# apple/ml-neuman

Measured on AMD Instinct MI355X. Metric: rays_per_sec (800x800 frame, 128 samples/ray coarse + 128 importance, NeuMan background NeRF), higher is better.
Workload: dtype coarse (sampling) pass: split-fp16 hi+lo MFMA x3, f32 accumulate; fine (shading) pass: per-row-scaled int16 as two int8 limbs on the i8 MFMA x3, exact int32 accumulate, encodings on split bf16

## Files before the change

ml-neuman_amd/csrc/mlp_host.hip:

```cpp
#include <stdarg.h>
#include <stdio.h>
#include <stdlib.h>
#include <string.h>

#include <vector>

#include "common.h"
#include "mlp_layout.h"
#include "mlp_launch.h"

namespace nm {

static thread_local char g_err[512] = "";

void set_error(const char* fmt, ...) {
    va_list ap;
    va_start(ap, fmt);
    vsnprintf(g_err, sizeof(g_err), fmt, ap);
    va_end(ap);
}
int check_hip(hipError_t e, const char* what) {
    if (e == hipSuccess) return NM_OK;
    set_error("%s: %s", what, hipGetErrorString(e));
    return NM_ERR_HIP;
// ... 278 lines not shown
                const float* row = hidden_row(d, P, st, n, &col0);
                float mx = 0.f;
                if (row) for (int f = 0; f < nh; ++f) mx = fmaxf(mx, fabsf(row[col0 + f] * uin[f]));
                q[n] = mx / (float)kFixedMax;
                kap = fmaxf(kap, q[n]);
            }
            if (!(kap > 0.f)) kap = 1.f;
            kappa[st] = kap;
            for (int n = 0; n < nrows; ++n) {
                if (!(q[n] > 0.f)) q[n] = kap;
                u[n] = q[n] / kap;
            }
            for (int nb = 0; nb < sh.nblk; ++nb)
                for (int r = 0; r < 32; ++r) {
                    const int n = 32 * nb + r;
                    int col0 = 0;
                    const float* row = hidden_row(d, P, st, n, &col0);
                    for (int t = 0; t < sh.i8steps; ++t) {
                        int8_t* hi = reinterpret_cast<int8_t*>(img + frag_off8(st, nb, t));
                        int8_t* lo = hi + 1024;
                        for (int g = 0; g < 2; ++g)
                            for (int e = 0; e < 16; ++e) {
                                const int f = slot_feature8(2 * t + g, e);
                                const float w = row ? row[col0 + f] * uin[f] : 0.f;
                                int v = (int)lrintf(w / q[n]);
                                if (v > kFixedMax) v = kFixedMax;
                                if (v < -kFixedMax) v = -kFixedMax;
                                const int l = ((v + 128) & 255) - 128;
                                const int h = (v - l) >> 8;
                                hi[(g * 32 + r) * 16 + e] = (int8_t)h;
                                lo[(g * 32 + r) * 16 + e] = (int8_t)l;
                            }
                    }
                }
        }
        for (int n = 0; n < nrows; ++n) b[n] /= u[n];
        for (int nb = 0; nb < sh.nblk; ++nb)
            for (int t = 0; t < sh.bfsteps; ++t) {
                uint16_t* hi = reinterpret_cast<uint16_t*>(img + frag_off8(st, nb, sh.i8steps + t));
                uint16_t* lo = hi + 64 * 8;
                const int cc0 = st == 9 ? 32 : 0;
                for (int lane = 0; lane < 64; ++lane)
                    for (int j = 0; j < 8; ++j) {
                        const int n = 32 * nb + (lane & 31);
                        const float wv = stage_weight(d, P, st, n, cc0 + 2 * t + (lane >> 5), j) / u[n];
                        const uint16_t h = f32_to_bf16(wv);
                        hi[lane * 8 + j] = h;
                        lo[lane * 8 + j] = f32_to_bf16(wv - bf16_to_f32(h));
                    }
            }
    }
}

static void pack_stream8s(const uint8_t* img8, uint8_t* out, bool plain = false) {
    memset(out, 0, (size_t)(kWeightBytes8 + kWeightPadBytes));
    uint8_t* dst = out;
    auto put = [&](int st, int nb, int t0, int n) {
        for (int t = 0; t < n; ++t, dst += kStepBytes) memcpy(dst, img8 + frag_off8(st, nb, t0 + t), (size_t)kStepBytes);
    };
    for (int nb = 0; nb < 8; ++nb) put(0, nb, 0, 4);
    for (int st = 1; st <= 7; ++st) {
        for (int nb = 0; nb < 8; ++nb) put(st, nb, 0, 8);
        if (st == 5)
            for (int nb = 0; nb < 8; ++nb) put(5, nb, 8, 4);
    }
    put(8, 8, 0, 8);
    if (plain) {
        for (int nb = 0; nb < 2; ++nb) { put(0, nb, 0, 4); dst += 4 * kStepBytes; }
        if (dst - out != kPlainStreamBytes8) abort();
        return;
    }
    for (int nb = 0; nb < 8; ++nb) put(8, nb, 0, 8);
    for (int nb = 0; nb < 4; ++nb) put(9, nb, 0, 10);
    put(10, 0, 0, 4);
    if (dst - out != kWeightBytes8) abort();
}

constexpr int kSigmaSteps = 8 * 4 + 6 * 8 * 16 + 8 * 20 + 16;
static void sigma_stream_table(std::vector<int>& tab, int ndir) {
    tab.clear();
    std::vector<int> direct;
    auto put = [&](int st, int b, int t0, int n) {
        for (int t = 0; t < n; ++t)
            for (int k = 0; k < 4; ++k) {
                const int off = (int)frag_off(st, b + (k >> 1), t0 + t) + 1024 * (k & 1);
                (k < 4 - ndir ? tab : direct).push_back(off);
            }
    };
    for (int st = 0; st <= 7; ++st) {
        const StageShape sh = stage_shape(st);
        for (int b = 0; b < 8; b += 2) {
            if (sh.pe_steps) put(st, b, 0, sh.pe_steps);
            for (int t0 = sh.pe_steps; t0 < sh.steps; t0 += 8) put(st, b, t0, 8);
        }
    }
    for (int t = 0; t < 16; ++t) { tab.push_back((int)frag_off(8, 8, t)); tab.push_back((int)frag_off(8, 8, t) + 1024); }
    tab.insert(tab.end(), direct.begin(), direct.end());
    if ((int)tab.size() != 2 * kSigmaSteps) abort();
}
__global__ void sigma_stream_kernel(const uint4* __restrict__ image, const int* __restrict__ tab, int npieces, uint4* __restrict__ out) {
    const int i = blockIdx.x * blockDim.x + threadIdx.x;
    if (i >= npieces * 64) return;
    out[i] = image[tab[i >> 6] / 16 + (i & 63)];
}

static void pack_stream8(const uint8_t* img8, uint8_t* out) {
    memset(out, 0, (size_t)kWeightBytes8w);
    for (int q = 0; q < 4; ++q) {
        uint8_t* dst = out + wstream_off(q);
        auto put = [&](int st, int nb, int t0, int n) {
            for (int t = 0; t < n; ++t, dst += kStepBytes) memcpy(dst, img8 + frag_off8(st, nb, t0 + t), (size_t)kStepBytes);
        };
        put(0, 2 * q, 0, 4); put(0, 2 * q + 1, 0, 4);
        for (int st = 1; st <= 8; ++st) {
            put(st, 2 * q, 0, 8); put(st, 2 * q + 1, 0, 8);
            if (st == 5) { put(5, 2 * q, 8, 4); put(5, 2 * q + 1, 8, 4); }
        }
        if (q < 2) put(8, 8, 0, 8);
        put(9, q, 0, 8); put(9, q, 8, 2);
        dst += 2 * kStepBytes;
        if (q < 2) put(10, 0, 0, 4);
        dst += kW8Pad * kStepBytes;
        if (dst != out + wstream_off(q) + (int64_t)wstream_steps(q) * kStepBytes) abort();
    }
}

}
// ... 41 lines not shown

int nm_mlp_pack_f16(const nm_mlp_desc* desc, const float* const* host_params, void* host_out) {
    if (int e = nm::validate_desc(desc)) return e;
    NM_REQUIRE(host_params && host_out, "nm_mlp_pack_f16: null pointer");
    for (int i = 0; i < (desc->plain_head ? 18 : 24); ++i) NM_REQUIRE(host_params[i], "nm_mlp_pack_f16: host_params[%d] is null", i);
    nm::pack_image(desc, host_params, static_cast<uint8_t*>(host_out), true);
    return NM_OK;
}

int64_t nm_mlp_pack_i8_bytes(const nm_mlp_desc* desc) {
    if (nm::validate_desc(desc) != NM_OK) return -1;
    return nm::image8_bytes();
}

int nm_mlp_pack_i8(const nm_mlp_desc* desc, const float* const* host_params, void* host_out) {
    if (int e = nm::validate_desc(desc)) return e;
    NM_REQUIRE(host_params && host_out, "nm_mlp_pack_i8: null pointer");
    for (int i = 0; i < (desc->plain_head ? 18 : 24); ++i) NM_REQUIRE(host_params[i], "nm_mlp_pack_i8: host_params[%d] is null", i);
    nm::pack_image8(desc, host_params, static_cast<uint8_t*>(host_out));
    return NM_OK;
}

int64_t nm_mlp_pack_i8s_bytes(const nm_mlp_desc* desc) {
    if (nm::validate_desc(desc) != NM_OK) return -1;
    return nm::kWeightBytes8 + nm::kWeightPadBytes;
}

int nm_mlp_pack_i8s(const nm_mlp_desc* desc, const float* const* host_params, void* host_out) {
    if (int e = nm::validate_desc(desc)) return e;
    NM_REQUIRE(host_params && host_out, "nm_mlp_pack_i8s: null pointer");
    for (int i = 0; i < (desc->plain_head ? 18 : 24); ++i) NM_REQUIRE(host_params[i], "nm_mlp_pack_i8s: host_params[%d] is null", i);
    std::vector<uint8_t> img8((size_t)nm::image8_bytes());
    nm::pack_image8(desc, host_params, img8.data());
    nm::pack_stream8s(img8.data(), static_cast<uint8_t*>(host_out), desc->plain_head != 0);
    return NM_OK;
}

int nm_mlp_create(const nm_mlp_desc* desc, const float* const* host_params, const float* host_pos_tab,
                  const float* host_dir_tab, nm_mlp_t* out) {
    if (int e = nm::validate_desc(desc)) return e;
    NM_REQUIRE(host_params && host_pos_tab && host_dir_tab && out, "nm_mlp_create: null pointer");
    const int plain = desc->plain_head;
    for (int i = 0; i < (plain ? 18 : 24); ++i) NM_REQUIRE(host_params[i], "nm_mlp_create: host_params[%d] is null", i);
    const int64_t bytes = nm_mlp_pack_bytes(desc);
    std::vector<uint8_t> img((size_t)bytes);
    nm::pack_image(desc, host_params, img.data());
    std::vector<uint8_t> img16((size_t)bytes);
    nm::pack_image(desc, host_params, img16.data(), true);
    std::vector<uint8_t> img8((size_t)nm::image8_bytes());
    std::vector<uint8_t> str8((size_t)nm::kWeightBytes8w);
    std::vector<uint8_t> str8s((size_t)(nm::kWeightBytes8 + nm::kWeightPadBytes));
    nm::pack_image8(desc, host_params, img8.data());
    nm::pack_stream8(img8.data(), str8.data());
    nm::pack_stream8s(img8.data(), str8s.data(), plain != 0);

    const int kpe = 3 + 6 * desc->pos_n_freqs, kdpe = 3 + 6 * desc->dir_n_freqs;
    const int K[12] = {kpe, 256, 256, 256, 256, kpe + 256, 256, 256, plain ? 0 : 256 + kdpe, plain ? 0 : 256, 256, plain ? 0 : 128};
    const int N[12] = {256, 256, 256, 256, 256, 256, 256, 256, plain ? 0 : 128, plain ? 0 : 256, plain ? 4 : 1, plain ? 0 : 3};
    const int src[12] = {0, 2, 4, 6, 8, 10, 12, 14, 16, 18, plain ? (int)nm::P_OUT_W : 20, 22};
    nm_mlp_s* m = new nm_mlp_s();
    m->desc = *desc;
    int woff = 0;
    for (int l = 0; l < 12; ++l) { m->ref_off[l] = woff; woff += K[l] * N[l]; }
    int boff = woff;
    for (int l = 0; l < 12; ++l) { m->ref_boff[l] = boff; boff += N[l]; }
    std::vector<float> ref((size_t)boff);
    for (int l = 0; l < 12; ++l) {
        if (!K[l]) continue;
        const float* W = host_params[src[l]];
        for (int k = 0; k < K[l]; ++k)
            for (int n = 0; n < N[l]; ++n) ref[m->ref_off[l] + (size_t)k * N[l] + n] = W[(size_t)n * K[l] + k];
        memcpy(&ref[m->ref_boff[l]], host_params[src[l] + 1], (size_t)N[l] * 4);
    }
    float tab[192];
    memset(tab, 0, sizeof(tab));
    const int npos = desc->pe_kind == NM_PE_POSENC ? desc->pos_n_freqs : 9 * desc->pos_n_freqs;
    const int ndir = desc->pe_kind == NM_PE_POSENC ? desc->dir_n_freqs : 9 * desc->dir_n_freqs;
    memcpy(tab, host_pos_tab, (size_t)npos * 4);
    memcpy(tab + 96, host_dir_tab, (size_t)ndir * 4);
    auto octaves = [&](const float* t, int nfreq) {
        const int per = desc->pe_kind == NM_PE_POSENC ? 1 : 9;
        for (int b = 0; b + 1 < nfreq; ++b)
            for (int k = 0; k < per; ++k)
                if (t[(b + 1) * per + k] != 2.f * t[b * per + k]) return 0;
        return 1;
    };
    m->pos_octaves = octaves(tab, desc->pos_n_freqs);
    m->dir_octaves = octaves(tab + 96, desc->dir_n_freqs);

    m->d_image = nullptr; m->d_image16 = nullptr; m->d_consts8 = nullptr; m->d_stream8 = nullptr; m->d_image8 = nullptr; m->d_stream16t = nullptr; m->d_sigma_tab = nullptr; m->d_bwd_image = nullptr; m->d_petab = nullptr; m->d_ref = nullptr; m->d_wscale16 = nullptr;
    int rc = nm::check_hip(hipMalloc(&m->d_image, (size_t)bytes), "nm_mlp_create: hipMalloc(image)");
    const size_t consts_off = (size_t)(nm::kWeightBytes8 + nm::kWeightPadBytes), consts_bytes = img8.size() - consts_off;
    if (!rc) rc = nm::check_hip(hipMalloc(&m->d_consts8, consts_bytes), "nm_mlp_create: hipMalloc(consts8)");
    if (!rc) rc = nm::check_hip(hipMemcpy(m->d_consts8, img8.data() + consts_off, consts_bytes, hipMemcpyHostToDevice), "nm_mlp_create: upload consts8");
    if (!rc) rc = nm::check_hip(hipMalloc(&m->d_stream8, str8.size()), "nm_mlp_create: hipMalloc(stream8)");
    if (!rc) rc = nm::check_hip(hipMemcpy(m->d_stream8, str8.data(), str8.size(), hipMemcpyHostToDevice), "nm_mlp_create: upload stream8");
    if (!rc) rc = nm::check_hip(hipMalloc(&m->d_image8, consts_off), "nm_mlp_create: hipMalloc(image8)");
    if (!rc) rc = nm::check_hip(hipMemcpy(m->d_image8, str8s.data(), consts_off, hipMemcpyHostToDevice), "nm_mlp_create: upload image8");
    if (!rc) rc = nm::check_hip(hipMalloc(&m->d_petab, sizeof(tab)), "nm_mlp_create: hipMalloc(petab)");
    if (!rc) rc = nm::check_hip(hipMalloc(&m->d_ref, ref.size() * 4), "nm_mlp_create: hipMalloc(ref)");
    if (!rc) rc = nm::check_hip(hipMemcpy(m->d_image, img.data(), (size_t)bytes, hipMemcpyHostToDevice), "nm_mlp_create: upload image");
    if (!rc) rc = nm::check_hip(hipMalloc(&m->d_image16, (size_t)bytes), "nm_mlp_create: hipMalloc(image16)");
    if (!rc) rc = nm::check_hip(hipMemcpy(m->d_image16, img16.data(), (size_t)bytes, hipMemcpyHostToDevice), "nm_mlp_create: upload image16");
    if (!rc) rc = nm::check_hip(hipMemcpy(m->d_petab, tab, sizeof(tab), hipMemcpyHostToDevice), "nm_mlp_create: upload petab");
    if (!rc) rc = nm::check_hip(hipMemcpy(m->d_ref, ref.data(), ref.size() * 4, hipMemcpyHostToDevice), "nm_mlp_create: upload ref");
    if (!rc && !plain) {
        std::vector<int> stab;
// ... 42 lines not shown
}

int nm_mlp_destroy(nm_mlp_t m) {
    if (!m) return NM_OK;
    if (m->d_image) (void)hipFree(m->d_image);
    if (m->d_image16) (void)hipFree(m->d_image16);
    if (m->d_consts8) (void)hipFree(m->d_consts8);
    if (m->d_stream8) (void)hipFree(m->d_stream8);
    if (m->d_image8) (void)hipFree(m->d_image8);
    if (m->d_stream16t) (void)hipFree(m->d_stream16t);
    if (m->d_sigma_tab) (void)hipFree(m->d_sigma_tab);
    if (m->d_bwd_image) (void)hipFree(m->d_bwd_image);
    if (m->d_petab) (void)hipFree(m->d_petab);
    if (m->d_ref) (void)hipFree(m->d_ref);
    if (m->d_wscale16) (void)hipFree(m->d_wscale16);
    delete m;
    return NM_OK;
}

static int mlp_dispatch(nm_mlp_t m, const float* pts, const float* dirs, const float* origin, const float* direction,
                        const float* z, int64_t n, int S, int in_mode, int precision, int stop_stage, float sigma_scale,
                        float* out, float* dbg, nm_stream_t stream, void* prof = nullptr, int sigma_only = 0,
                        const nm::MlpChunk* chunk = nullptr) {
    NM_REQUIRE(m, "nm_mlp_forward: null handle");
    NM_REQUIRE(n >= 0, "nm_mlp_forward: negative n");
    NM_REQUIRE(precision == NM_PREC_FP32 || precision == NM_PREC_BF16X3 || precision == NM_PREC_BF16 || precision == NM_PREC_I8X3 ||
                   precision == NM_PREC_FP16X3,
               "nm_mlp_forward: bad precision %d", precision);
    if (n == 0) return NM_OK;
    NM_REQUIRE(!(chunk && precision == NM_PREC_FP32), "nm_mlp_forward_ray_chunk: the exact-f32 validation kernel has no chunked form");
    NM_REQUIRE(!(m->desc.plain_head && precision == NM_PREC_I8X3 && (stop_stage != -2 || dbg || prof || sigma_only)),
               "nm_mlp_forward: the plain-head (use_viewdirs=False) net's i8x3 form is the whole-network launch only (no stage-by-stage / density-only form)");
    NM_REQUIRE(!(m->desc.plain_head && stop_stage > 7), "nm_mlp_forward_debug: the plain-head net has stages -1..7 only");
    if (precision == NM_PREC_FP32) {
        nm::RefLaunch L;
        L.plain_head = m->desc.plain_head;
        L.wt = m->d_ref; L.bias = m->d_ref; L.petab = m->d_petab;
        for (int i = 0; i < 12; ++i) { L.off[i] = m->ref_off[i]; L.boff[i] = m->ref_boff[i]; }
        L.pe_kind = m->desc.pe_kind; L.pos_nfreq = m->desc.pos_n_freqs; L.dir_nfreq = m->desc.dir_n_freqs;
        return nm::launch_mlp_ref(L, pts, dirs, origin, direction, z, n, S, in_mode, stop_stage, sigma_scale, out, dbg,
                                  nm::as_stream(stream));
    }
    nm::MlpLaunch L;
    L.wpack = m->d_image;
    L.bias = reinterpret_cast<const float*>(m->d_image + nm::kWeightBytes + nm::kWeightPadBytes);
    L.wpack16 = m->d_image16;
    L.bias16 = reinterpret_cast<const float*>(m->d_image16 + nm::kWeightBytes + nm::kWeightPadBytes);
    L.petab = m->d_petab;
    L.pe_kind = m->desc.pe_kind; L.pos_nfreq = m->desc.pos_n_freqs; L.dir_nfreq = m->desc.dir_n_freqs;
    L.pos_octaves = m->pos_octaves; L.dir_octaves = m->dir_octaves;
    L.plain_head = m->desc.plain_head;
    L.wstream8 = m->d_stream8;
    L.consts8 = m->d_consts8;
    static const bool i8_as = [] { const char* e = getenv("NEUMAN_I8_KERNEL"); return !e || !strcmp(e, "as"); }();
    const char* sk = getenv("NEUMAN_SIGMA_KERNEL");
    const bool sigma_t = !(sk && !strcmp(sk, "w")) && m->d_stream16t;
    if (sigma_t && precision == NM_PREC_FP16X3 && sigma_only == 1 && stop_stage == -2 && !dbg && !prof && !m->desc.plain_head)
        return nm::launch_sigma_f16t(L, m->d_stream16t, m->sigma_ndir, pts, dirs, origin, direction, z, n, S, in_mode, sigma_scale, out, nm::as_stream(stream), chunk, nullptr, -1);
    if ((i8_as || m->desc.plain_head) && precision == NM_PREC_I8X3 && stop_stage == -2 && !dbg && !prof && !sigma_only)
        return nm::launch_mlp_i8s(L, m->d_image8, pts, dirs, origin, direction, z, n, S, in_mode, sigma_scale, out, nm::as_stream(stream), chunk);
    return nm::launch_mlp_mfma(L, pts, dirs, origin, direction, z, n, S, in_mode, precision, stop_stage, sigma_scale, out, dbg,
                               prof, nm::as_stream(stream), sigma_only, chunk);
}

int nm_mlp_forward(nm_mlp_t mlp, const float* pts, const float* dirs, int64_t n, int precision, float sigma_scale,
                   float* out, nm_stream_t stream) {
    NM_REQUIRE(n == 0 || (pts && dirs && out), "nm_mlp_forward: null pointer");
    NM_REQUIRE((reinterpret_cast<uintptr_t>(out) & 15) == 0, "nm_mlp_forward: out must be 16-byte aligned");
    return mlp_dispatch(mlp, pts, dirs, nullptr, nullptr, nullptr, n, 1, 0, precision, -2, sigma_scale, out, nullptr, stream);
}

int nm_mlp_forward_save(nm_mlp_t m, const float* pts, const float* dirs, int64_t n, float* save_h, float* save_hv, float* out,
                        nm_stream_t stream) {
    return nm_mlp_forward_save_bits(m, pts, dirs, n, save_h, save_hv, nullptr, out, stream);
}

static int forward_save_impl(nm_mlp_t m, const float* pts, const float* dirs, int64_t n, float* save_h, float* save_hv, uint32_t* save_bits,
                             void* save_h16, float* out, nm_stream_t stream, void* save_feat16 = nullptr, uint32_t* save_hvbits = nullptr,
                             void* save_x0h = nullptr, void* save_d0h = nullptr) {
    NM_REQUIRE(m, "nm_mlp_forward_save: null handle");
    NM_REQUIRE(n >= 0, "nm_mlp_forward_save: negative n");
    if (n == 0) return NM_OK;
    const bool plain = m->desc.plain_head != 0;
    NM_REQUIRE(!plain || (save_h16 && !save_h && !save_feat16 && !save_hvbits && !save_d0h), "nm_mlp_forward_save: the plain-head net keeps save_h16 / save_bits / save_x0h only");
    NM_REQUIRE(pts && (dirs || plain) && (plain || ((save_h || (save_h16 && save_feat16)) && save_hv)) && out, "nm_mlp_forward_save: null pointer");
    NM_REQUIRE(((reinterpret_cast<uintptr_t>(out) | reinterpret_cast<uintptr_t>(save_h) | reinterpret_cast<uintptr_t>(save_hv) | reinterpret_cast<uintptr_t>(save_h16) |
                 reinterpret_cast<uintptr_t>(save_feat16)) & 15) == 0, "nm_mlp_forward_save: outputs must be 16-byte aligned");
    nm::MlpLaunch L;
    L.wpack = m->d_image;
    L.bias = reinterpret_cast<const float*>(m->d_image + nm::kWeightBytes + nm::kWeightPadBytes);
    L.wpack16 = m->d_image16;
    L.bias16 = reinterpret_cast<const float*>(m->d_image16 + nm::kWeightBytes + nm::kWeightPadBytes);
    L.petab = m->d_petab;
    L.pe_kind = m->desc.pe_kind; L.pos_nfreq = m->desc.pos_n_freqs; L.dir_nfreq = m->desc.dir_n_freqs;
    L.pos_octaves = m->pos_octaves; L.dir_octaves = m->dir_octaves;
    L.plain_head = plain ? 1 : 0;
    L.wstream8 = m->d_stream8;
    L.consts8 = m->d_consts8;
    L.save_h = save_h; L.save_hv = save_hv; L.save_bits = save_bits; L.save_h16 = save_h16; L.save_feat16 = save_feat16; L.save_hvbits = save_hvbits; L.save_x0h = save_x0h; L.save_d0h = save_d0h;
    return nm::launch_mlp_mfma(L, pts, dirs ? dirs : pts, nullptr, nullptr, nullptr, n, 1, 0, NM_PREC_FP16X3, -2, 1.f, out, nullptr, nullptr,
                               nm::as_stream(stream), 0, nullptr);
}

int nm_mlp_forward_save_bits(nm_mlp_t m, const float* pts, const float* dirs, int64_t n, float* save_h, float* save_hv, uint32_t* save_bits,
                             float* out, nm_stream_t stream) {
    return forward_save_impl(m, pts, dirs, n, save_h, save_hv, save_bits, nullptr, out, stream);
}

int nm_mlp_forward_save16(nm_mlp_t m, const float* pts, const float* dirs, int64_t n, uint16_t* save_h16, float* save_feat, uint16_t* save_feat16,
                          float* save_hv, uint32_t* save_bits, uint32_t* save_hvbits, uint16_t* save_x0h, uint16_t* save_d0h, float* out, nm_stream_t stream) {
    NM_REQUIRE(n == 0 || (save_h16 && save_bits && (save_feat || save_feat16 || (m && m->desc.plain_head))), "nm_mlp_forward_save16: null pointer");
    NM_REQUIRE(((reinterpret_cast<uintptr_t>(save_x0h) | reinterpret_cast<uintptr_t>(save_d0h)) & 15) == 0, "nm_mlp_forward_save16: outputs must be 16-byte aligned");
    return forward_save_impl(m, pts, dirs, n, save_feat, save_hv, save_bits, save_h16, out, stream, save_feat16, save_hvbits, save_x0h, save_d0h);
// ... 226 lines not shown
```

ml-neuman_amd/csrc/mlp_i8s.hip:

```cpp
#include "mlp_i8as.h"
#include <stdio.h>
#include <stdlib.h>
#include <vector>

namespace {

constexpr int kWaves = 8;
constexpr int kTile = kWaves * kRows;
constexpr int kPWaveU4 = nm::kPeChunks * 2 * kRows;
constexpr int kPeU4 = kWaves * kPWaveU4;
constexpr int kStepU4 = nm::kStepBytes / 16;
constexpr int kSlotU4 = 12 * kStepU4;
constexpr int kSlots = 3;
constexpr int kBiasU4 = (nm::kBiasFloats + 16 + 3) / 4;
constexpr int kTileBlocks = 82;
__host__ __device__ constexpr int block_steps(int i) {
    i = i >= kTileBlocks ? i - kTileBlocks : i;
    return i < 8 ? 4 : i < 77 ? 8 : i < 81 ? 10 : 4;
}
__host__ __device__ constexpr int block_pieces(int nsteps) { return (2 * nsteps + kWaves - 1) / kWaves; }

#ifdef NM_AS_PROF
struct Prof {
    unsigned long long t, acc[8];
};
#define PROF_DECL Prof P; P.t = __builtin_amdgcn_s_memtime(); for (int i_ = 0; i_ < 8; ++i_) P.acc[i_] = 0;
#define PROF_TICK(b) { const unsigned long long n_ = __builtin_amdgcn_s_memtime(); P.acc[b] += n_ - P.t; P.t = n_; }
#define PROF_ARG , Prof& P
#define PROF_PASS , P
#else
#define PROF_DECL
#define PROF_TICK(b)
#define PROF_ARG
#define PROF_PASS
#endif
struct Ring {
    const char* src;
    const uint4* rd;
    unsigned lds0;
    int off;
    int slot;
    int refill, np, nsteps2;
};
__device__ __forceinline__ void ring_piece(const Ring& R, int off, int slot, int j) {
    glds16(R.src + off + j * (kWaves * 1024), __builtin_amdgcn_readfirstlane(R.lds0 + slot * (kSlotU4 * 16) + j * (kWaves * 1024)));
}
__device__ __forceinline__ void ring_advance(Ring& R, int nsteps) {
    R.off += nsteps * nm::kStepBytes;
    if (R.off == (int)nm::kWeightBytes8) R.off = 0;
}
__device__ __forceinline__ const uint4* ring_enter(Ring& R, int i PROF_ARG) {
    PROF_TICK(4)
    const int np1 = block_pieces(block_steps(i + 1));
    if (np1 == 1) asm volatile("s_waitcnt vmcnt(1)" ::: "memory");
    else if (np1 == 2) asm volatile("s_waitcnt vmcnt(2)" ::: "memory");
    else asm volatile("s_waitcnt vmcnt(3)" ::: "memory");
    __builtin_amdgcn_s_barrier();
    PROF_TICK(0)
    const uint4* cur = R.rd + R.slot * kSlotU4;
    R.refill = R.slot == 0 ? kSlots - 1 : R.slot - 1;
    R.slot = R.slot == kSlots - 1 ? 0 : R.slot + 1;
    R.np = block_pieces(block_steps(i + 2));
    R.nsteps2 = block_steps(i + 2);
    return cur;
}
__device__ __forceinline__ void ring_copy(Ring& R, int j) {
    if (j < R.np) ring_piece(R, R.off, R.refill, j);
    if (j == R.np - 1) ring_advance(R, R.nsteps2);
}
struct W8 {
    uint4 h, l;
};

template <int NSTEPS, bool PEND, bool RELU = true>
__device__ __forceinline__ void k_i8_impl(i32x16& t, const X8& X, const uint4* ws, Ring& R, f32x16& fp, const i32x16& tp, lds_cfloat* bias_blk,
                                          float sx256, float& m) {
    i32x16 ah, ac;
#pragma unroll
    for (int r = 0; r < 16; ++r) { ah[r] = 0; ac[r] = 0; }
    W8 w[2];
    w[0].h = ws[0]; w[0].l = ws[64];
    w[1].h = ws[kStepU4]; w[1].l = ws[kStepU4 + 64];
#pragma unroll
    for (int s = 0; s < NSTEPS; ++s) {
        const uint4 wh = w[s & 1].h, wl = w[s & 1].l;
        ac = __builtin_amdgcn_mfma_i32_32x32x32_i8(as_i32x4(wh), as_i32x4(X.l[s]), ac, 0, 0, 0);
        ah = __builtin_amdgcn_mfma_i32_32x32x32_i8(as_i32x4(wh), as_i32x4(X.h[s]), ah, 0, 0, 0);
        ac = __builtin_amdgcn_mfma_i32_32x32x32_i8(as_i32x4(wl), as_i32x4(X.h[s]), ac, 0, 0, 0);
        if (s + 2 < NSTEPS) { w[s & 1].h = ws[(s + 2) * kStepU4]; w[s & 1].l = ws[(s + 2) * kStepU4 + 64]; }
        if (s == 0 || s == 2 || s == 4) ring_copy(R, s >> 1);
        if (PEND) {
            const int r = 2 * s;
            const float b0 = bias_blk[8 * (r >> 2) + (r & 3)], b1 = bias_blk[8 * (r >> 2) + (r & 3) + 1];
            const float f0 = fmaf((float)tp[r], sx256, b0), f1 = fmaf((float)tp[r + 1], sx256, b1);
            fp[r] = f0;
            fp[r + 1] = f1;
            m = RELU ? fmaxf(m, fmaxf(f0, f1)) : fmaxf(m, fmaxf(fabsf(f0), fabsf(f1)));
            __builtin_amdgcn_sched_barrier(0);
        }
    }
#pragma unroll
    for (int r = 0; r < 16; ++r) t[r] = (ah[r] << 8) + ac[r];
}
template <int NSTEPS>
__device__ __forceinline__ void k_i8(i32x16& t, const X8& X, const uint4* ws, Ring& R) {
    f32x16 nf;
    float nm_ = 0.f;
    k_i8_impl<NSTEPS, false>(t, X, ws, R, nf, t, nullptr, 0.f, nm_);
}
template <int NSTEPS, bool COPY = false>
__device__ __forceinline__ void k_bf(f32x16& f, const uint4* pw, int g, int s, const uint4* ws, Ring* R = nullptr, int j0 = 0) {
#pragma unroll
    for (int t = 0; t < NSTEPS; ++t) {
        if (COPY && (t == 1 || t == 3)) ring_copy(*R, j0 + (t >> 1));
        const uint4 wh = ws[t * kStepU4], wl = ws[t * kStepU4 + 64];
        const uint4 xh = pw[(2 * t + g) * (2 * kRows) + s], xl = pw[(2 * t + g) * (2 * kRows) + kRows + s];
        f = __builtin_amdgcn_mfma_f32_32x32x16_bf16(as_bf16x8(wh), as_bf16x8(xl), f, 0, 0, 0);
        f = __builtin_amdgcn_mfma_f32_32x32x16_bf16(as_bf16x8(wl), as_bf16x8(xh), f, 0, 0, 0);
        f = __builtin_amdgcn_mfma_f32_32x32x16_bf16(as_bf16x8(wh), as_bf16x8(xh), f, 0, 0, 0);
    }
}
template <bool PLAIN>
__global__ __launch_bounds__(kWaves * 64, 2) void nerf_mlp_i8s_kernel(const Args8s A) {
    __shared__ uint4 lds[kPeU4 + kSlots * kSlotU4 + kBiasU4];
    const MlpArgs a = resolve_args(A.a);
    const int tid = threadIdx.x, lane = tid & 63;
    const int w = __builtin_amdgcn_readfirstlane(tid >> 6);
    const int g = lane >> 5, s = lane & 31;
    uint4* pw = lds + w * kPWaveU4;
    Ring R;
    R.src = reinterpret_cast<const char*>(A.image8) + lane * 16 + w * 1024;
    R.rd = lds + kPeU4 + lane;
    R.lds0 = (unsigned)(uintptr_t)(lds + kPeU4) + w * 1024;
    R.off = 0;
    R.slot = 0;
    {
        float* lb = reinterpret_cast<float*>(lds + kPeU4 + kSlots * kSlotU4);
        for (int i = tid; i < nm::kBiasFloats + 16; i += kWaves * 64) lb[i] = A.consts8[nm::kBiasFloats + i];
    }
    __syncthreads();
    ring_piece(R, 0, 0, 0);
    ring_piece(R, block_steps(0) * nm::kStepBytes, 1, 0);
    R.off = (block_steps(0) + block_steps(1)) * nm::kStepBytes;
    const float u_sigma = A.consts8[nm::stage_b_off(8) + 256];
    const float u_r = A.consts8[nm::stage_b_off(10)], u_g = A.consts8[nm::stage_b_off(10) + 1], u_b = A.consts8[nm::stage_b_off(10) + 2];
    const float* kappa = reinterpret_cast<const float*>(lds + kPeU4 + kSlots * kSlotU4) + nm::kBiasFloats;
    unsigned bias_lds = (unsigned)(uintptr_t)(lds + kPeU4 + kSlots * kSlotU4) + 16 * g;
    asm volatile("" : "+v"(bias_lds));
    lds_cfloat* bias = (lds_cfloat*)(uintptr_t)bias_lds;
    const int64_t ntiles = (a.n + kTile - 1) / kTile;
    for (int i = lane; i < kPWaveU4; i += 64) pw[i] = make_uint4(0, 0, 0, 0);
    PROF_DECL

#pragma unroll 1
    for (int64_t tile = blockIdx.x; tile < ntiles; tile += gridDim.x) {
        const int64_t row0 = tile * kTile + w * kRows;
        PROF_TICK(7)
        fill_pe_wave(pw, false, a, row0, lane);
        PROF_TICK(6)
        X8 X;
        float sx;
        {
            f32x16 f[8];
            float m = 0.f;
#pragma unroll
            for (int b = 0; b < 8; ++b) {
                const uint4* ws = ring_enter(R, b PROF_PASS);
                bias16(f[b], bias + nm::stage_b_off(0) + 32 * b);
                k_bf<4, true>(f[b], pw, g, s, ws, &R);
                PROF_TICK(2)
                m = max16<true>(m, f[b]);
            }
            PROF_TICK(4)
            const float M = row_max(m), inv = inv_of(M);
#pragma unroll
            for (int b = 0; b < 8; ++b) quant16<true>(f[b], inv, X.h[b], X.l[b]);
            sx = scale_of(M);
            PROF_TICK(5)
        }
#pragma unroll 1
        for (int st = 1; st <= 7; ++st) {
            const float sxin = sx * (256.f * kappa[st]);
            const int i0 = 8 * st + (st > 5 ? 4 : 0);
            f32x16 f[8];
            float m = 0.f;
            i32x16 tp;
#pragma unroll
            for (int b = 0; b < 8; ++b) {
                const uint4* ws = ring_enter(R, i0 + b PROF_PASS);
                if (b == 0) {
                    k_i8<8>(tp, X, ws, R);
                } else {
                    i32x16 t;
                    k_i8_impl<8, true>(t, X, ws, R, f[b - 1], tp, bias + 256 * st + 32 * (b - 1), sxin, m);
                    tp = t;
                }
                PROF_TICK(2)
            }
            dequant16(f[7], tp, sxin, bias + 256 * st + 32 * 7);
            if (st == 5) {
#pragma unroll
                for (int u = 0; u < 4; ++u) {
                    const uint4* ws = ring_enter(R, 48 + u PROF_PASS);
                    k_bf<4, true>(f[2 * u], pw, g, s, ws, &R, 0);
                    k_bf<4, true>(f[2 * u + 1], pw, g, s, ws + 4 * kStepU4, &R, 2);
                    PROF_TICK(2)
                }
                m = 0.f;
#pragma unroll
                for (int b = 0; b < 7; ++b) m = max16<true>(m, f[b]);
            }
            m = max16<true>(m, f[7]);
            PROF_TICK(4)
            const float M = row_max(m), inv = inv_of(M);
#pragma unroll
            for (int b = 0; b < 8; ++b) quant16<true>(f[b], inv, X.h[b], X.l[b]);
            sx = scale_of(M);
            PROF_TICK(5)
            if (st == 5 && !(PLAIN && a.sigma_only == 2)) {
                PROF_TICK(7)
                fill_pe_wave(pw, true, a, row0, lane);
                PROF_TICK(6)
            }
        }
        if (PLAIN && a.sigma_only == 2) {
            i32x16 t;
            f32x16 fo;
            k_i8<8>(t, X, ring_enter(R, 68 PROF_PASS), R);
            PROF_TICK(2)
            dequant16(fo, t, sx * (256.f * kappa[8]), bias + nm::stage_b_off(8) + 256);
            const float* up = A.consts8 + nm::stage_b_off(8) + 256;
            const int64_t i = row0 + s;
            if (g == 0 && i < a.n)
                reinterpret_cast<float4*>(a.out)[sample_record(a, i)] = make_float4(fo[0] * up[0], fo[1] * up[1], fo[2] * up[2], fo[3] * up[3] * a.sigma_scale);
            R.off = (block_steps(0) + block_steps(1)) * nm::kStepBytes;
            continue;
        }
        float sigma;
        {
            const float sxin = sx * (256.f * kappa[8]);
            {
                i32x16 t;
                f32x16 fa;
                k_i8<8>(t, X, ring_enter(R, 68 PROF_PASS), R);
                PROF_TICK(2)
                dequant16(fa, t, sxin, bias + nm::stage_b_off(8) + 256);
                sigma = fa[0] * u_sigma;
            }
            f32x16 f[8];
            float m = 0.f;
#pragma unroll
            for (int b = 0; b < 8; ++b) {
                i32x16 t;
                k_i8<8>(t, X, ring_enter(R, 69 + b PROF_PASS), R);
                PROF_TICK(2)
                dequant16(f[b], t, sxin, bias + nm::stage_b_off(8) + 32 * b);
                m = max16<false>(m, f[b]);
            }
            PROF_TICK(4)
            const float M = row_max(m), inv = inv_of(M);
#pragma unroll
            for (int b = 0; b < 8; ++b) quant16<false>(f[b], inv, X.h[b], X.l[b]);
            sx = scale_of(M);
            PROF_TICK(5)
        }
        {
            const float sxin = sx * (256.f * kappa[9]);
            f32x16 f[4];
            float m = 0.f;
#pragma unroll
            for (int b = 0; b < 4; ++b) {
                i32x16 t;
                const uint4* ws = ring_enter(R, 77 + b PROF_PASS);
                k_i8<8>(t, X, ws, R);
                PROF_TICK(2)
                dequant16(f[b], t, sxin, bias + nm::stage_b_off(9) + 32 * b);
                k_bf<2>(f[b], pw, g, s, ws + 8 * kStepU4);
                m = max16<true>(m, f[b]);
            }
            PROF_TICK(4)
            const float M = row_max(m), inv = inv_of(M);
#pragma unroll
            for (int b = 0; b < 4; ++b) quant16<true>(f[b], inv, X.h[b], X.l[b]);
            sx = scale_of(M);
            PROF_TICK(5)
        }
        {
            i32x16 t;
            f32x16 fr;
            k_i8<4>(t, X, ring_enter(R, 81 PROF_PASS), R);
            PROF_TICK(2)
            dequant16(fr, t, sx * (256.f * kappa[10]), bias + nm::stage_b_off(10));
            const int64_t i = row0 + s;
            if (g == 0 && i < a.n)
                reinterpret_cast<float4*>(a.out)[sample_record(a, i)] =
                    make_float4(fr[0] * u_r, fr[1] * u_g, fr[2] * u_b,
                                sigma * a.sigma_scale);
        }
    }
#ifdef NM_AS_PROF
    PROF_TICK(7)
    if (lane == 0 && a.prof)
        for (int i = 0; i < 8; ++i) a.prof[((size_t)blockIdx.x * kWaves + w) * 8 + i] = P.acc[i];
#endif
    asm volatile("s_waitcnt vmcnt(0)" ::: "memory");
}

}

namespace nm {

int launch_mlp_i8s(const MlpLaunch& L, const void* image8, const float* pts, const float* dirs, const float* origin, const float* direction,
                   const float* z, int64_t n, int S, int in_mode, float sigma_scale, float* out, hipStream_t stream, const MlpChunk* chunk) {
    Args8s A;
    MlpArgs& a = A.a;
    a.ray_idx = chunk ? chunk->ray_idx : nullptr;
    a.n_rays_dev = chunk ? chunk->n_rays_dev : nullptr;
    a.s0 = chunk ? chunk->s0 : 0;
    a.S_total = chunk ? chunk->S_total : S;
    a.wpack = nullptr; a.bias = nullptr;
    a.petab = L.petab;
    a.pts = pts; a.dirs = dirs; a.origin = origin; a.direction = direction; a.z = z;
    a.out = out; a.dbg = nullptr; a.prof = nullptr; a.n = n; a.S = S; a.in_mode = in_mode; a.stop_stage = -2; a.sigma_scale = sigma_scale;
    a.sigma_only = L.plain_head ? 2 : 0;
    a.save_h = nullptr; a.save_hv = nullptr; a.save_bits = nullptr; a.save_h16 = nullptr; a.save_feat16 = nullptr; a.save_hvbits = nullptr; a.save_x0h = nullptr; a.save_d0h = nullptr;
    a.pos = PeSpec{L.pe_kind, L.pos_nfreq, L.pos_octaves};
    a.dir = PeSpec{L.pe_kind, L.dir_nfreq, L.dir_octaves};
    A.consts8 = L.consts8;
    A.image8 = reinterpret_cast<const uint4*>(image8);
    const int64_t ntiles = (n + kTile - 1) / kTile;
    int dev = 0, cus = 256;
    if (hipGetDevice(&dev) == hipSuccess) {
        int v = 0;
        if (hipDeviceGetAttribute(&v, hipDeviceAttributeMultiprocessorCount, dev) == hipSuccess && v > 0) cus = v;
    }
    const int grid = (int)(ntiles < cus ? ntiles : cus);
    if (getenv("NEUMAN_I8S_DEBUG")) {
        int nb = -1;
        hipError_t e = hipOccupancyMaxActiveBlocksPerMultiprocessor(&nb, nerf_mlp_i8s_kernel<false>, kWaves * 64, 0);
        fprintf(stderr, "nerf_mlp_i8s_kernel: occupancy %d blocks/CU (%s), grid %d, cus %d\n", nb, hipGetErrorString(e), grid, cus);
    }
#ifdef NM_AS_PROF
    static unsigned long long* d_prof = nullptr;
    const size_t nprof = (size_t)grid * kWaves * 8;
    if (!d_prof) (void)hipMalloc(&d_prof, (size_t)1024 * kWaves * 8 * 8);
    (void)hipMemsetAsync(d_prof, 0, nprof * 8, stream);
    a.prof = d_prof;
#endif
    if (L.plain_head) hipLaunchKernelGGL(nerf_mlp_i8s_kernel<true>, dim3(grid), dim3(kWaves * 64), 0, stream, A);
    else hipLaunchKernelGGL(nerf_mlp_i8s_kernel<false>, dim3(grid), dim3(kWaves * 64), 0, stream, A);
#ifdef NM_AS_PROF
    if (n > 1000000) {
        std::vector<unsigned long long> h(nprof);
        (void)hipStreamSynchronize(stream);
        (void)hipMemcpy(h.data(), d_prof, nprof * 8, hipMemcpyDeviceToHost);
        static const char* names[8] = {"top barrier", "copy issue", "k-loop", "-", "epilogue", "requantise", "encodings", "rest"};
        double acc[8] = {0}, tot = 0;
        for (size_t i = 0; i < nprof; ++i) acc[i & 7] += (double)h[i];
        for (int i = 0; i < 8; ++i) tot += acc[i];
        fprintf(stderr, "mean cycles per wave %.0f:", tot / (grid * (double)kWaves));
        for (int i = 0; i < 8; ++i) fprintf(stderr, "  %s %.1f%%", names[i], 100.0 * acc[i] / tot);
        fprintf(stderr, "\n");
    }
#endif
    return check_launch("nerf_mlp_i8s_kernel");
}

}
```

ml-neuman_amd/csrc/mlp_launch.h:

```cpp
#pragma once
#include "common.h"

namespace nm {

enum { P_OUT_W = 16, P_OUT_B = 17 };
enum { P_PTS_W = 0, P_VIEWS_W = 16, P_VIEWS_B = 17, P_FEAT_W = 18, P_FEAT_B = 19, P_ALPHA_W = 20, P_ALPHA_B = 21, P_RGB_W = 22, P_RGB_B = 23 };
struct DevParams {
    const float* p[24];
};

struct MlpLaunch {
    const void* wpack; const float* bias; const float* petab;
    int pe_kind, pos_nfreq, dir_nfreq;
    int pos_octaves, dir_octaves;
    int plain_head;
    const void* wpack16; const float* bias16;
    const void* wstream8; const float* consts8;
    float* save_h = nullptr;
    float* save_hv = nullptr;
    unsigned* save_bits = nullptr;
    void* save_h16 = nullptr;
    void* save_feat16 = nullptr;
    unsigned* save_hvbits = nullptr;
    void* save_x0h = nullptr; void* save_d0h = nullptr;
};
struct RefLaunch {
    const float* wt; const float* bias; int off[12]; int boff[12]; const float* petab;
    int pe_kind, pos_nfreq, dir_nfreq;
    int plain_head;
};

struct MlpChunk {
    const int* ray_idx; const int* n_rays_dev; int s0, S_total;
};

int launch_mlp_mfma(const MlpLaunch& L, const float* pts, const float* dirs, const float* origin, const float* direction,
                    const float* z, int64_t n, int S, int in_mode, int precision, int stop_stage, float sigma_scale, float* out,
                    float* dbg, void* prof, hipStream_t stream, int sigma_only = 0, const MlpChunk* chunk = nullptr);
int launch_mlp_i8s(const MlpLaunch& L, const void* image8, const float* pts, const float* dirs, const float* origin, const float* direction,
                   const float* z, int64_t n, int S, int in_mode, float sigma_scale, float* out, hipStream_t stream, const MlpChunk* chunk);
int sigma_f16t_ndir();
int launch_sigma_f16t(const MlpLaunch& L, const void* stream16t, int stream_ndir, const float* pts, const float* dirs, const float* origin, const float* direction,
                      const float* z, int64_t n, int S, int in_mode, float sigma_scale, float* out, hipStream_t stream, const MlpChunk* chunk,
                      float* dbg, int dbg_stage);
int64_t mlp_bwd_image_bytes();
struct Bwd16 {
    void* dz16; void* dfeat16; const float* amax; float* dz32[8];
    const unsigned* hvbits = nullptr; void* dhv16 = nullptr; float* dhv32 = nullptr; int kdir = 0;
    int plain = 0;
};
int launch_mlp_bwd(const DevParams& P, int kpe, uint8_t* image, const float* dz_top, const float* d_feat, const float* d_raw, const float* acts,
                   const unsigned* relu_bits, int64_t n, float* dz_out, float* colsum, float* gb, hipStream_t stream, const Bwd16* h = nullptr);
int launch_mlp_ref(const RefLaunch& L, const float* pts, const float* dirs, const float* origin, const float* direction,
                   const float* z, int64_t n, int S, int in_mode, int stop_stage, float sigma_scale, float* out, float* dbg,
                   hipStream_t stream);

}
```

Before: 1.471 million.

## Use 16x16x64 i8 MFMA tiles in the fine shading kernel by default

Adds a K16 variant of the int8 shading kernel that replaces each 32x32x32 i8 MFMA triple with 16x16x64 i8 MFMAs. Weights are re-cut on the host into the matching fragment layout, and activations and accumulators are moved between lanes with permlane16_swap. This variant becomes the default when NEUMAN_I8_KERNEL is unset or set to "as". The aim is higher i8 MFMA throughput or better issue behaviour from the 16x16x64 shape. In exchange it adds lane-swap instructions, more accumulator registers and a fragile host-side layout permutation.

```diff
diff --git a/ml-neuman_amd/csrc/mlp_host.hip b/ml-neuman_amd/csrc/mlp_host.hip
--- a/ml-neuman_amd/csrc/mlp_host.hip
+++ b/ml-neuman_amd/csrc/mlp_host.hip
@@ -354,27 +354,54 @@
     }
 }
 
-static void pack_stream8s(const uint8_t* img8, uint8_t* out, bool plain = false) {
+static int i8s_kernel() {
+    static const int k = [] {
+        const char* e = getenv("NEUMAN_I8_KERNEL");
+        return !e || !strcmp(e, "as") ? 16 : !strcmp(e, "as32") ? 32 : 0;
+    }();
+    return k;
+}
+
+static void recut_stream8s16(uint8_t* blk, int n) {
+    std::vector<uint8_t> src(blk, blk + (size_t)n * kStepBytes);
+    for (int kk = 0; kk < n / 2; ++kk)
+        for (int fh = 0; fh < 2; ++fh)
+            for (int limb = 0; limb < 2; ++limb)
+                for (int l = 0; l < 64; ++l) {
+                    const int q = l >> 4, m = l & 15;
+                    const int r = (m & 3) | (((m >> 3) & 1) << 2) | (((m >> 2) & 1) << 3);
+                    const int L = 16 * fh + r + 32 * (q >> 1);
+                    memcpy(blk + (size_t)(2 * kk + fh) * kStepBytes + limb * 1024 + l * 16,
+                           src.data() + (size_t)(2 * kk + (q & 1)) * kStepBytes + limb * 1024 + L * 16, 16);
+                }
+}
+
+static void pack_stream8s(const uint8_t* img8, uint8_t* out, bool plain = false, bool k16 = false) {
     memset(out, 0, (size_t)(kWeightBytes8 + kWeightPadBytes));
     uint8_t* dst = out;
     auto put = [&](int st, int nb, int t0, int n) {
         for (int t = 0; t < n; ++t, dst += kStepBytes) memcpy(dst, img8 + frag_off8(st, nb, t0 + t), (size_t)kStepBytes);
     };
+    auto put8 = [&](int st, int nb, int n) {
+        uint8_t* d0 = dst;
+        put(st, nb, 0, n);
+        if (k16) recut_stream8s16(d0, n);
+    };
     for (int nb = 0; nb < 8; ++nb) put(0, nb, 0, 4);
     for (int st = 1; st <= 7; ++st) {
-        for (int nb = 0; nb < 8; ++nb) put(st, nb, 0, 8);
+        for (int nb = 0; nb < 8; ++nb) put8(st, nb, 8);
         if (st == 5)
             for (int nb = 0; nb < 8; ++nb) put(5, nb, 8, 4);
     }
-    put(8, 8, 0, 8);
+    put8(8, 8, 8);
     if (plain) {
         for (int nb = 0; nb < 2; ++nb) { put(0, nb, 0, 4); dst += 4 * kStepBytes; }
         if (dst - out != kPlainStreamBytes8) abort();
         return;
     }
-    for (int nb = 0; nb < 8; ++nb) put(8, nb, 0, 8);
-    for (int nb = 0; nb < 4; ++nb) put(9, nb, 0, 10);
-    put(10, 0, 0, 4);
+    for (int nb = 0; nb < 8; ++nb) put8(8, nb, 8);
+    for (int nb = 0; nb < 4; ++nb) { put8(9, nb, 8); put(9, nb, 8, 2); }
+    put8(10, 0, 4);
     if (dst - out != kWeightBytes8) abort();
 }
 
@@ -522,7 +549,7 @@
     std::vector<uint8_t> str8s((size_t)(nm::kWeightBytes8 + nm::kWeightPadBytes));
     nm::pack_image8(desc, host_params, img8.data());
     nm::pack_stream8(img8.data(), str8.data());
-    nm::pack_stream8s(img8.data(), str8s.data(), plain != 0);
+    nm::pack_stream8s(img8.data(), str8s.data(), plain != 0, nm::i8s_kernel() == 16);
 
     const int kpe = 3 + 6 * desc->pos_n_freqs, kdpe = 3 + 6 * desc->dir_n_freqs;
     const int K[12] = {kpe, 256, 256, 256, 256, kpe + 256, 256, 256, plain ? 0 : 256 + kdpe, plain ? 0 : 256, 256, plain ? 0 : 128};
@@ -671,13 +698,14 @@
     L.plain_head = m->desc.plain_head;
     L.wstream8 = m->d_stream8;
     L.consts8 = m->d_consts8;
-    static const bool i8_as = [] { const char* e = getenv("NEUMAN_I8_KERNEL"); return !e || !strcmp(e, "as"); }();
+    const bool i8_as = nm::i8s_kernel() != 0;
     const char* sk = getenv("NEUMAN_SIGMA_KERNEL");
     const bool sigma_t = !(sk && !strcmp(sk, "w")) && m->d_stream16t;
     if (sigma_t && precision == NM_PREC_FP16X3 && sigma_only == 1 && stop_stage == -2 && !dbg && !prof && !m->desc.plain_head)
         return nm::launch_sigma_f16t(L, m->d_stream16t, m->sigma_ndir, pts, dirs, origin, direction, z, n, S, in_mode, sigma_scale, out, nm::as_stream(stream), chunk, nullptr, -1);
     if ((i8_as || m->desc.plain_head) && precision == NM_PREC_I8X3 && stop_stage == -2 && !dbg && !prof && !sigma_only)
-        return nm::launch_mlp_i8s(L, m->d_image8, pts, dirs, origin, direction, z, n, S, in_mode, sigma_scale, out, nm::as_stream(stream), chunk);
+        return nm::launch_mlp_i8s(L, m->d_image8, pts, dirs, origin, direction, z, n, S, in_mode, sigma_scale, out, nm::as_stream(stream), chunk,
+                                  nm::i8s_kernel() == 16);
     return nm::launch_mlp_mfma(L, pts, dirs, origin, direction, z, n, S, in_mode, precision, stop_stage, sigma_scale, out, dbg,
                                prof, nm::as_stream(stream), sigma_only, chunk);
 }
diff --git a/ml-neuman_amd/csrc/mlp_i8s.hip b/ml-neuman_amd/csrc/mlp_i8s.hip
--- a/ml-neuman_amd/csrc/mlp_i8s.hip
+++ b/ml-neuman_amd/csrc/mlp_i8s.hip
@@ -5,6 +5,7 @@
 
 namespace {
 
+typedef __attribute__((ext_vector_type(2))) unsigned u32x2;
 constexpr int kWaves = 8;
 constexpr int kTile = kWaves * kRows;
 constexpr int kPWaveU4 = nm::kPeChunks * 2 * kRows;
@@ -72,21 +73,32 @@
     uint4 h, l;
 };
 
-template <int NSTEPS, bool PEND, bool RELU = true>
+template <int NSTEPS, bool PEND, bool RELU = true, bool K16 = false>
 __device__ __forceinline__ void k_i8_impl(i32x16& t, const X8& X, const uint4* ws, Ring& R, f32x16& fp, const i32x16& tp, lds_cfloat* bias_blk,
                                           float sx256, float& m) {
     i32x16 ah, ac;
-#pragma unroll
-    for (int r = 0; r < 16; ++r) { ah[r] = 0; ac[r] = 0; }
+    i32x4 bh[2][2], bc[2][2];
+#pragma unroll
+    for (int r = 0; r < 16; ++r) { ah[r] = 0; ac[r] = 0; bh[r >> 3][(r >> 2) & 1][r & 3] = 0; bc[r >> 3][(r >> 2) & 1][r & 3] = 0; }
     W8 w[2];
     w[0].h = ws[0]; w[0].l = ws[64];
     w[1].h = ws[kStepU4]; w[1].l = ws[kStepU4 + 64];
 #pragma unroll
     for (int s = 0; s < NSTEPS; ++s) {
         const uint4 wh = w[s & 1].h, wl = w[s & 1].l;
-        ac = __builtin_amdgcn_mfma_i32_32x32x32_i8(as_i32x4(wh), as_i32x4(X.l[s]), ac, 0, 0, 0);
-        ah = __builtin_amdgcn_mfma_i32_32x32x32_i8(as_i32x4(wh), as_i32x4(X.h[s]), ah, 0, 0, 0);
-        ac = __builtin_amdgcn_mfma_i32_32x32x32_i8(as_i32x4(wl), as_i32x4(X.h[s]), ac, 0, 0, 0);
+        if (K16) {
+            const int kk = s >> 1, fh = s & 1;
+#pragma unroll
+            for (int sh = 0; sh < 2; ++sh) bc[fh][sh] = __builtin_amdgcn_mfma_i32_16x16x64_i8(as_i32x4(wh), as_i32x4(X.l[2 * kk + sh]), bc[fh][sh], 0, 0, 0);
+#pragma unroll
+            for (int sh = 0; sh < 2; ++sh) bh[fh][sh] = __builtin_amdgcn_mfma_i32_16x16x64_i8(as_i32x4(wh), as_i32x4(X.h[2 * kk + sh]), bh[fh][sh], 0, 0, 0);
+#pragma unroll
+            for (int sh = 0; sh < 2; ++sh) bc[fh][sh] = __builtin_amdgcn_mfma_i32_16x16x64_i8(as_i32x4(wl), as_i32x4(X.h[2 * kk + sh]), bc[fh][sh], 0, 0, 0);
+        } else {
+            ac = __builtin_amdgcn_mfma_i32_32x32x32_i8(as_i32x4(wh), as_i32x4(X.l[s]), ac, 0, 0, 0);
+            ah = __builtin_amdgcn_mfma_i32_32x32x32_i8(as_i32x4(wh), as_i32x4(X.h[s]), ah, 0, 0, 0);
+            ac = __builtin_amdgcn_mfma_i32_32x32x32_i8(as_i32x4(wl), as_i32x4(X.h[s]), ac, 0, 0, 0);
+        }
         if (s + 2 < NSTEPS) { w[s & 1].h = ws[(s + 2) * kStepU4]; w[s & 1].l = ws[(s + 2) * kStepU4 + 64]; }
         if (s == 0 || s == 2 || s == 4) ring_copy(R, s >> 1);
         if (PEND) {
@@ -99,14 +111,43 @@
             __builtin_amdgcn_sched_barrier(0);
         }
     }
-#pragma unroll
-    for (int r = 0; r < 16; ++r) t[r] = (ah[r] << 8) + ac[r];
-}
-template <int NSTEPS>
+    if (K16) {
+#pragma unroll
+        for (int fh = 0; fh < 2; ++fh)
+#pragma unroll
+            for (int r = 0; r < 4; ++r) {
+                const u32x2 sw = __builtin_amdgcn_permlane16_swap((unsigned)((bh[fh][0][r] << 8) + bc[fh][0][r]), (unsigned)((bh[fh][1][r] << 8) + bc[fh][1][r]), false, false);
+                t[8 * fh + r] = (int)sw.x;
+                t[8 * fh + 4 + r] = (int)sw.y;
+            }
+    } else {
+#pragma unroll
+        for (int r = 0; r < 16; ++r) t[r] = (ah[r] << 8) + ac[r];
+    }
+}
+template <bool K16, int NSTEPS = 8>
+__device__ __forceinline__ void to_b16(X8& X) {
+    if (!K16) return;
+#pragma unroll
+    for (int kk = 0; kk < NSTEPS / 2; ++kk) {
+        unsigned* h0 = reinterpret_cast<unsigned*>(&X.h[2 * kk]);
+        unsigned* h1 = reinterpret_cast<unsigned*>(&X.h[2 * kk + 1]);
+        unsigned* l0 = reinterpret_cast<unsigned*>(&X.l[2 * kk]);
+        unsigned* l1 = reinterpret_cast<unsigned*>(&X.l[2 * kk + 1]);
+#pragma unroll
+        for (int d = 0; d < 4; ++d) {
+            const u32x2 a = __builtin_amdgcn_permlane16_swap(h0[d], h1[d], false, false);
+            h0[d] = a.x; h1[d] = a.y;
+            const u32x2 b = __builtin_amdgcn_permlane16_swap(l0[d], l1[d], false, false);
+            l0[d] = b.x; l1[d] = b.y;
+        }
+    }
+}
+template <int NSTEPS, bool K16>
 __device__ __forceinline__ void k_i8(i32x16& t, const X8& X, const uint4* ws, Ring& R) {
     f32x16 nf;
     float nm_ = 0.f;
-    k_i8_impl<NSTEPS, false>(t, X, ws, R, nf, t, nullptr, 0.f, nm_);
+    k_i8_impl<NSTEPS, false, true, K16>(t, X, ws, R, nf, t, nullptr, 0.f, nm_);
 }
 template <int NSTEPS, bool COPY = false>
 __device__ __forceinline__ void k_bf(f32x16& f, const uint4* pw, int g, int s, const uint4* ws, Ring* R = nullptr, int j0 = 0) {
@@ -120,7 +161,7 @@
         f = __builtin_amdgcn_mfma_f32_32x32x16_bf16(as_bf16x8(wh), as_bf16x8(xh), f, 0, 0, 0);
     }
 }
-template <bool PLAIN>
+template <bool PLAIN, bool K16>
 __global__ __launch_bounds__(kWaves * 64, 2) void nerf_mlp_i8s_kernel(const Args8s A) {
     __shared__ uint4 lds[kPeU4 + kSlots * kSlotU4 + kBiasU4];
     const MlpArgs a = resolve_args(A.a);
@@ -175,6 +216,7 @@
             const float M = row_max(m), inv = inv_of(M);
 #pragma unroll
             for (int b = 0; b < 8; ++b) quant16<true>(f[b], inv, X.h[b], X.l[b]);
+            to_b16<K16>(X);
             sx = scale_of(M);
             PROF_TICK(5)
         }
@@ -189,10 +231,10 @@
             for (int b = 0; b < 8; ++b) {
                 const uint4* ws = ring_enter(R, i0 + b PROF_PASS);
                 if (b == 0) {
-                    k_i8<8>(tp, X, ws, R);
+                    k_i8<8, K16>(tp, X, ws, R);
                 } else {
                     i32x16 t;
-                    k_i8_impl<8, true>(t, X, ws, R, f[b - 1], tp, bias + 256 * st + 32 * (b - 1), sxin, m);
+                    k_i8_impl<8, true, true, K16>(t, X, ws, R, f[b - 1], tp, bias + 256 * st + 32 * (b - 1), sxin, m);
                     tp = t;
                 }
                 PROF_TICK(2)
@@ -215,6 +257,7 @@
             const float M = row_max(m), inv = inv_of(M);
 #pragma unroll
             for (int b = 0; b < 8; ++b) quant16<true>(f[b], inv, X.h[b], X.l[b]);
+            to_b16<K16>(X);
             sx = scale_of(M);
             PROF_TICK(5)
             if (st == 5 && !(PLAIN && a.sigma_only == 2)) {
@@ -226,7 +269,7 @@
         if (PLAIN && a.sigma_only == 2) {
             i32x16 t;
             f32x16 fo;
-            k_i8<8>(t, X, ring_enter(R, 68 PROF_PASS), R);
+            k_i8<8, K16>(t, X, ring_enter(R, 68 PROF_PASS), R);
             PROF_TICK(2)
             dequant16(fo, t, sx * (256.f * kappa[8]), bias + nm::stage_b_off(8) + 256);
             const float* up = A.consts8 + nm::stage_b_off(8) + 256;
@@ -242,7 +285,7 @@
             {
                 i32x16 t;
                 f32x16 fa;
-                k_i8<8>(t, X, ring_enter(R, 68 PROF_PASS), R);
+                k_i8<8, K16>(t, X, ring_enter(R, 68 PROF_PASS), R);
                 PROF_TICK(2)
                 dequant16(fa, t, sxin, bias + nm::stage_b_off(8) + 256);
                 sigma = fa[0] * u_sigma;
@@ -252,7 +295,7 @@
 #pragma unroll
             for (int b = 0; b < 8; ++b) {
                 i32x16 t;
-                k_i8<8>(t, X, ring_enter(R, 69 + b PROF_PASS), R);
+                k_i8<8, K16>(t, X, ring_enter(R, 69 + b PROF_PASS), R);
                 PROF_TICK(2)
                 dequant16(f[b], t, sxin, bias + nm::stage_b_off(8) + 32 * b);
                 m = max16<false>(m, f[b]);
@@ -261,6 +304,7 @@
             const float M = row_max(m), inv = inv_of(M);
 #pragma unroll
             for (int b = 0; b < 8; ++b) quant16<false>(f[b], inv, X.h[b], X.l[b]);
+            to_b16<K16>(X);
             sx = scale_of(M);
             PROF_TICK(5)
         }
@@ -272,7 +316,7 @@
             for (int b = 0; b < 4; ++b) {
                 i32x16 t;
                 const uint4* ws = ring_enter(R, 77 + b PROF_PASS);
-                k_i8<8>(t, X, ws, R);
+                k_i8<8, K16>(t, X, ws, R);
                 PROF_TICK(2)
                 dequant16(f[b], t, sxin, bias + nm::stage_b_off(9) + 32 * b);
                 k_bf<2>(f[b], pw, g, s, ws + 8 * kStepU4);
@@ -282,13 +326,14 @@
             const float M = row_max(m), inv = inv_of(M);
 #pragma unroll
             for (int b = 0; b < 4; ++b) quant16<true>(f[b], inv, X.h[b], X.l[b]);
+            to_b16<K16, 4>(X);
             sx = scale_of(M);
             PROF_TICK(5)
         }
         {
             i32x16 t;
             f32x16 fr;
-            k_i8<4>(t, X, ring_enter(R, 81 PROF_PASS), R);
+            k_i8<4, K16>(t, X, ring_enter(R, 81 PROF_PASS), R);
             PROF_TICK(2)
             dequant16(fr, t, sx * (256.f * kappa[10]), bias + nm::stage_b_off(10));
             const int64_t i = row0 + s;
@@ -311,7 +356,7 @@
 namespace nm {
 
 int launch_mlp_i8s(const MlpLaunch& L, const void* image8, const float* pts, const float* dirs, const float* origin, const float* direction,
-                   const float* z, int64_t n, int S, int in_mode, float sigma_scale, float* out, hipStream_t stream, const MlpChunk* chunk) {
+                   const float* z, int64_t n, int S, int in_mode, float sigma_scale, float* out, hipStream_t stream, const MlpChunk* chunk, bool k16) {
     Args8s A;
     MlpArgs& a = A.a;
     a.ray_idx = chunk ? chunk->ray_idx : nullptr;
@@ -337,8 +382,8 @@
     const int grid = (int)(ntiles < cus ? ntiles : cus);
     if (getenv("NEUMAN_I8S_DEBUG")) {
         int nb = -1;
-        hipError_t e = hipOccupancyMaxActiveBlocksPerMultiprocessor(&nb, nerf_mlp_i8s_kernel<false>, kWaves * 64, 0);
-        fprintf(stderr, "nerf_mlp_i8s_kernel: occupancy %d blocks/CU (%s), grid %d, cus %d\n", nb, hipGetErrorString(e), grid, cus);
+        hipError_t e = hipOccupancyMaxActiveBlocksPerMultiprocessor(&nb, k16 ? nerf_mlp_i8s_kernel<false, true> : nerf_mlp_i8s_kernel<false, false>, kWaves * 64, 0);
+        fprintf(stderr, "nerf_mlp_i8s_kernel<%s>: occupancy %d blocks/CU (%s), grid %d, cus %d\n", k16 ? "16x16" : "32x32", nb, hipGetErrorString(e), grid, cus);
     }
 #ifdef NM_AS_PROF
     static unsigned long long* d_prof = nullptr;
@@ -347,8 +392,13 @@
     (void)hipMemsetAsync(d_prof, 0, nprof * 8, stream);
     a.prof = d_prof;
 #endif
-    if (L.plain_head) hipLaunchKernelGGL(nerf_mlp_i8s_kernel<true>, dim3(grid), dim3(kWaves * 64), 0, stream, A);
-    else hipLaunchKernelGGL(nerf_mlp_i8s_kernel<false>, dim3(grid), dim3(kWaves * 64), 0, stream, A);
+    if (k16) {
+        if (L.plain_head) hipLaunchKernelGGL((nerf_mlp_i8s_kernel<true, true>), dim3(grid), dim3(kWaves * 64), 0, stream, A);
+        else hipLaunchKernelGGL((nerf_mlp_i8s_kernel<false, true>), dim3(grid), dim3(kWaves * 64), 0, stream, A);
+    } else {
+        if (L.plain_head) hipLaunchKernelGGL((nerf_mlp_i8s_kernel<true, false>), dim3(grid), dim3(kWaves * 64), 0, stream, A);
+        else hipLaunchKernelGGL((nerf_mlp_i8s_kernel<false, false>), dim3(grid), dim3(kWaves * 64), 0, stream, A);
+    }
 #ifdef NM_AS_PROF
     if (n > 1000000) {
         std::vector<unsigned long long> h(nprof);
diff --git a/ml-neuman_amd/csrc/mlp_launch.h b/ml-neuman_amd/csrc/mlp_launch.h
--- a/ml-neuman_amd/csrc/mlp_launch.h
+++ b/ml-neuman_amd/csrc/mlp_launch.h
@@ -38,7 +38,8 @@
                     const float* z, int64_t n, int S, int in_mode, int precision, int stop_stage, float sigma_scale, float* out,
                     float* dbg, void* prof, hipStream_t stream, int sigma_only = 0, const MlpChunk* chunk = nullptr);
 int launch_mlp_i8s(const MlpLaunch& L, const void* image8, const float* pts, const float* dirs, const float* origin, const float* direction,
-                   const float* z, int64_t n, int S, int in_mode, float sigma_scale, float* out, hipStream_t stream, const MlpChunk* chunk);
+                   const float* z, int64_t n, int S, int in_mode, float sigma_scale, float* out, hipStream_t stream, const MlpChunk* chunk,
+                   bool k16);
 int sigma_f16t_ndir();
 int launch_sigma_f16t(const MlpLaunch& L, const void* stream16t, int stream_ndir, const float* pts, const float* dirs, const float* origin, const float* direction,
                       const float* z, int64_t n, int S, int in_mode, float sigma_scale, float* out, hipStream_t stream, const MlpChunk* chunk,
```

Result: no change. 1.483 million, median of 6 (+0.8%).
